# intel/hexl

Hardware: NVIDIA H100
Metric: ntt_per_sec_fwd_inv_N65536_q55_batch8192 (higher is better)
Workload: dtype u64

## Files before the change

### hexl_b200/csrc/ntt.cu

```cuda
#include "ntt_kernels.cuh"

namespace hexl_b200 {
namespace {

template <int MODE, int LOGC>
cudaError_t launch_row(bool fwd, const NttDeviceTables& t, u64* result, const u64* operand,
                       u64 batch, int out_mf, int fold, cudaStream_t stream) {
  using Cfg = RowCfg<LOGC, MODE>;
  const unsigned rows_per_poly = (unsigned)(t.n >> LOGC);
  const u64 total_rows = batch * rows_per_poly;
  const unsigned grid = (unsigned)((total_rows + Cfg::ROWS - 1) / Cfg::ROWS);
  const Mod m = make_mod(t);
  if (fwd) {
    if (cudaError_t e = ensure_dynamic_smem<ntt_row_fwd<MODE, LOGC>>(Cfg::SMEM)) return e;
    ntt_row_fwd<MODE, LOGC><<<grid, Cfg::THREADS, Cfg::SMEM, stream>>>(result, operand, Tab<MODE>::fwd(t), m,
                                                                       total_rows, rows_per_poly, out_mf);
  } else {
    if (cudaError_t e = ensure_dynamic_smem<ntt_row_inv<MODE, LOGC>>(Cfg::SMEM)) return e;
    ntt_row_inv<MODE, LOGC><<<grid, Cfg::THREADS, Cfg::SMEM, stream>>>(
        result, operand, Tab<MODE>::inv(t), m, total_rows, rows_per_poly, out_mf, fold, Tab<MODE>::inv_n(t),
        Tab<MODE>::inv_n_w(t));
  }
  count_launch();
  return cudaGetLastError();
// ... 22 lines not shown
  const unsigned grid = (unsigned)((total_cols + threads - 1) / threads);
  const Mod m = make_mod(t);
  if (fwd)
    ntt_col<MODE, LOGR, true><<<grid, threads, 0, stream>>>(result, operand, Tab<MODE>::fwd(t), m, t.log_n, log_s,
                                                            total_cols, out_mf, fold, Tab<MODE>::inv_n(t),
                                                            Tab<MODE>::inv_n_w(t));
  else
    ntt_col<MODE, LOGR, false><<<grid, threads, 0, stream>>>(result, operand, Tab<MODE>::inv(t), m, t.log_n, log_s,
                                                             total_cols, out_mf, fold, Tab<MODE>::inv_n(t),
                                                             Tab<MODE>::inv_n_w(t));
  count_launch();
  return cudaGetLastError();
}

template <int MODE>
cudaError_t launch_col_dyn(int log_r, bool fwd, const NttDeviceTables& t, u64* result,
                           const u64* operand, u64 batch, int log_s, int out_mf, int fold,
                           cudaStream_t stream) {
  switch (log_r) {
    case 3: return launch_col<MODE, 3>(fwd, t, result, operand, batch, log_s, out_mf, fold, stream);
    case 4: return launch_col<MODE, 4>(fwd, t, result, operand, batch, log_s, out_mf, fold, stream);
  }
  if constexpr (MODE != kSmall)
    if (log_r == 5) return launch_col<MODE, 5>(fwd, t, result, operand, batch, log_s, out_mf, fold, stream);
  return cudaErrorInvalidValue;
}

cudaError_t simple_transform(bool fwd, const NttDeviceTables& t, u64* result, const u64* operand,
                             int out_mf, u64 batch, cudaStream_t stream) {
  const u64 total = batch << (t.log_n - 1);
  const unsigned threads = 128, grid = (unsigned)((total + threads - 1) / threads);
  const u64* src = operand;
  const Mod m = make_mod(t);
  for (int k = 0; k < t.log_n; ++k) {
    const int s = fwd ? k : t.log_n - 1 - k;
    const int last = k == t.log_n - 1;
    if (fwd)
      ntt_stage_simple<true><<<grid, threads, 0, stream>>>(result, src, t.fwd, m, t.log_n, s, total,
                                                           out_mf, last, t.inv_n, t.inv_n_w);
    else
      ntt_stage_simple<false><<<grid, threads, 0, stream>>>(result, src, t.inv, m, t.log_n, s, total,
                                                            out_mf, last, t.inv_n, t.inv_n_w);
    count_launch();
    src = result;
  }
  return cudaGetLastError();
}

template <int MODE, int LOGR>
cudaError_t launch_fused(bool fwd, const NttDeviceTables& t, u64* result, const u64* operand, u64 batch,
                         int out_mf, cudaStream_t stream) {
  using Cfg = FusedCfg<LOGR>;
  const Mod m = make_mod(t);
  cudaLaunchConfig_t cfg = {};
  cfg.gridDim = dim3((unsigned)(batch * Cfg::K));
  cfg.blockDim = dim3(Cfg::THREADS);
  cfg.dynamicSmemBytes = Cfg::SMEM;
  cfg.stream = stream;
  cudaLaunchAttribute attr;
  attr.id = cudaLaunchAttributeClusterDimension;
  attr.val.clusterDim.x = Cfg::K;
  attr.val.clusterDim.y = 1;
  attr.val.clusterDim.z = 1;
  cfg.attrs = &attr;
  cfg.numAttrs = 1;
  cudaError_t e;
  if (fwd)
    e = cudaLaunchKernelEx(&cfg, ntt_fused_fwd<MODE, LOGR>, result, operand, Tab<MODE>::fwd(t), m, out_mf);
  else
    e = cudaLaunchKernelEx(&cfg, ntt_fused_inv<MODE, LOGR>, result, operand, Tab<MODE>::inv(t), m, out_mf,
                           Tab<MODE>::inv_n(t), Tab<MODE>::inv_n_w(t));
  count_launch();
  return e != cudaSuccess ? e : cudaGetLastError();
}

template <int MODE, int LOGR>
cudaError_t launch_pipe(const NttDeviceTables& t, u64* result, const u64* operand, u64 batch, int out_mf,
                        cudaStream_t stream) {
  return launch_pipelined<ntt_pipe_fwd<MODE, LOGR>, PipeCfg<LOGR>>(batch, stream, result, operand, Tab<MODE>::fwd(t),
                                                                  make_mod(t), out_mf);
}

template <int MODE, int LOGR>
cudaError_t launch_dsmem(bool fwd, const NttDeviceTables& t, u64* result, const u64* operand, u64 batch, int out_mf,
                         cudaStream_t stream) {
  using Cfg = DsmemCfg<LOGR, MODE>;
  const Mod m = make_mod(t);
  cudaLaunchConfig_t cfg = {};
  cfg.gridDim = dim3((unsigned)(batch * Cfg::K));
  cfg.blockDim = dim3(Cfg::THREADS);
  cfg.dynamicSmemBytes = Cfg::SMEM;
  cfg.stream = stream;
  cudaLaunchAttribute attr;
  attr.id = cudaLaunchAttributeClusterDimension;
  attr.val.clusterDim.x = Cfg::K;
  attr.val.clusterDim.y = 1;
  attr.val.clusterDim.z = 1;
  cfg.attrs = &attr;
  cfg.numAttrs = 1;
  cudaError_t e;
  if (fwd) {
    if ((e = ensure_dynamic_smem<ntt_dsmem_fwd<MODE, LOGR>>(Cfg::SMEM)) != cudaSuccess) return e;
    e = cudaLaunchKernelEx(&cfg, ntt_dsmem_fwd<MODE, LOGR>, result, operand, Tab<MODE>::fwd(t), m, out_mf);
  } else {
    if ((e = ensure_dynamic_smem<ntt_dsmem_inv<MODE, LOGR>>(Cfg::SMEM)) != cudaSuccess) return e;
    e = cudaLaunchKernelEx(&cfg, ntt_dsmem_inv<MODE, LOGR>, result, operand, Tab<MODE>::inv(t), m, out_mf,
                           Tab<MODE>::inv_n(t), Tab<MODE>::inv_n_w(t));
  }
  count_launch();
  return e != cudaSuccess ? e : cudaGetLastError();
}

enum : int { kSplit, kPipe, kFused, kDsmem };
struct SinglePass {
  int kernel, log_r;
};
template <int MODE>
SinglePass plan_single_pass(int log_n, u64 batch, bool forward) {
  const int lr = log_n - 12;
  if (lr < 2 || lr > 5) return {kSplit, 0};
  if (MODE == kSmall) return {kDsmem, lr};
  if (forward && lr >= 3 && batch >= 64 && batch < (1ull << 31)) return {kPipe, lr};
  if (lr <= 3) return {kDsmem, lr};
  if (lr == 4) return {kFused, lr};
// ... 96 lines not shown
```

### hexl_b200/csrc/ntt_kernels.cuh

```cuda
#pragma once
#include <algorithm>
#include <atomic>
#include <cstdio>
#include <cstdlib>

#include "internal.h"

namespace hexl_b200 {
namespace {

template <int I>
struct Idx {
  __host__ __device__ constexpr operator int() const { return I; }
};
template <int BEGIN, int END, typename F>
__device__ __forceinline__ void static_for(F&& f) {
  if constexpr (BEGIN < END) {
    f(Idx<BEGIN>{});
    static_for<BEGIN + 1, END>(f);
  }
}

enum : int { kGeneric = 0, kFast = 1, kSmall = 2, kWide = 3 };

// ... 146 lines not shown
  return join(t0, t1);
}

template <int MODE, typename TW>
__device__ __forceinline__ void fwd_bfly(u64& X, u64& Y, const TW& w, const Mod& m) {
  if (MODE == kFast) {
    const u64 T = mul_tw<kFast>(Y, w, m);
    Y = X + m.four_q - T;
    X = add_alu(X, T, m);
  } else if (MODE == kWide) {
    const u64 tx = csub(X, m.four_q);
    const u64 T = mul_tw<kWide>(Y, w, m);
    X = add_alu(tx, T, m);
    Y = tx + m.four_q - T;
  } else {
    const u64 tx = csub_s(X, m.two_q);
    const u64 T = mul_tw<kGeneric>(Y, w, m);
    X = tx + T;
    Y = tx + m.two_q - T;
  }
}

template <int MODE, typename TW>
__device__ __forceinline__ void inv_bfly(u64& X, u64& Y, const TW& w, const Mod& m, u64 cq) {
  if (MODE == kFast) {
    const u64 d = X + cq - Y;
    X = add_alu(X, Y, m);
    Y = mul_tw<kFast>(d, w, m);
  } else if (MODE == kWide) {
    const u64 s = add_alu(X, Y, m);
    const u64 d = X + m.four_q - Y;
    X = csub_s(s, m.four_q);
    Y = mul_tw<kWide>(d, w, m);
  } else {
    const u64 s = X + Y;
    const u64 d = X + m.two_q - Y;
    X = csub_s(s, m.two_q);
    Y = mul_tw<kGeneric>(d, w, m);
  }
}

template <int MODE>
__device__ __forceinline__ void inv_bfly_last(u64& X, u64& Y, const Twiddle inv_n, const Twiddle inv_n_w,
                                              const Mod& m, u64 cq) {
  const u64 s = add_alu(X, Y, m);
  const u64 d = X + cq - Y;
  if (MODE == kFast || MODE == kWide) {
    X = mul_tw<MODE>(s, inv_n, m);
    Y = mul_tw<MODE>(d, inv_n_w, m);
  } else {
    X = mul_tw_exact(s, inv_n, m);
    Y = mul_tw_exact(d, inv_n_w, m);
  }
}

template <int MODE>
__device__ __forceinline__ u64 fwd_out(u64 v, const Mod& m, int out_mf) {
  if (MODE == kFast) v = barrett_lazy3_bigq(v, m);
  if (MODE == kWide) v = csub_s(v, m.four_q);
  return out_mf == 1 ? csub_s(csub_s(v, m.two_q), m.q) : v;
}
template <int MODE>
__device__ __forceinline__ u64 inv_out(u64 v, const Mod& m, int out_mf) {
  if (MODE == kFast || MODE == kWide) v = csub_s(v, m.two_q);
  return out_mf == 1 ? csub_s(v, m.q) : v;
}

__device__ __forceinline__ unsigned csub32(unsigned x, unsigned c) { return min(x, x - c); }
__device__ __forceinline__ unsigned mul_tw32(unsigned x, const Twiddle32 w, const Mod& m) {
  const unsigned Q = hi32(mul_wide(x, w.wp));
  return mad_lo(Q, m.n0, x * w.w);
}
template <int MODE, typename TW>
__device__ __forceinline__ void fwd_bfly(unsigned& X, unsigned& Y, const TW& w, const Mod& m) {
  const unsigned two_q = lo32(m.two_q);
  const unsigned tx = csub32(X, two_q);
  const unsigned T = mul_tw32(Y, w, m);
  X = tx + T;
  Y = tx + two_q - T;
}
template <int MODE, typename TW>
__device__ __forceinline__ void inv_bfly(unsigned& X, unsigned& Y, const TW& w, const Mod& m, unsigned) {
  const unsigned two_q = lo32(m.two_q);
  const unsigned s = X + Y;
  const unsigned d = X + two_q - Y;
  X = csub32(s, two_q);
  Y = mul_tw32(d, w, m);
}
template <int MODE>
__device__ __forceinline__ void inv_bfly_last(unsigned& X, unsigned& Y, const Twiddle32 inv_n,
                                              const Twiddle32 inv_n_w, const Mod& m, unsigned) {
  const unsigned s = X + Y;
  const unsigned d = X + lo32(m.two_q) - Y;
  X = mul_tw32(s, inv_n, m);
  Y = mul_tw32(d, inv_n_w, m);
}
template <int MODE>
__device__ __forceinline__ unsigned fwd_out(unsigned v, const Mod& m, int out_mf) {
  return out_mf == 1 ? csub32(csub32(v, lo32(m.two_q)), lo32(m.q)) : v;
}
template <int MODE>
__device__ __forceinline__ unsigned inv_out(unsigned v, const Mod& m, int out_mf) {
  return out_mf == 1 ? csub32(v, lo32(m.q)) : v;
}

__host__ __device__ constexpr int inv_slot_bound(int K, int low) {
// ... 311 lines not shown
        static_for<0, 16>([&](auto I) {
          constexpr int e = I;
          mir->p[p][mir->off + reg_index<LB0>(u, e)] = (u64)inv_out<MODE>(v[e], m, out_mf);
        });
      }
    }
  }
}

template <int MODE, int LOGC>
__global__ void __launch_bounds__(RowCfg<LOGC, MODE>::THREADS, RowCfg<LOGC, MODE>::MIN_BLOCKS)
    ntt_row_fwd(u64* result, const u64* operand, const typename Ar<MODE>::Tw* __restrict__ tw, const Mod m,
                u64 total_rows, unsigned rows_per_poly, int out_mf) {
  using Cfg = RowCfg<LOGC, MODE>;
  extern __shared__ __align__(16) unsigned char smem[];
  const unsigned row_local = threadIdx.x / Cfg::T, u = threadIdx.x % Cfg::T;
  u64 row = (u64)blockIdx.x * Cfg::ROWS + row_local;
  const bool active = row < total_rows;
  if (!active) row = total_rows - 1;
  const u64 base = (u64)rows_per_poly + (row % rows_per_poly);
  typename Cfg::Tw* cta_stab = nullptr;
  if (MODE == kSmall && Cfg::ROWS > 1 && Cfg::TW_TABLES && rows_per_poly == 1)
    cta_stab = reinterpret_cast<typename Cfg::Tw*>(smem + (size_t)row_elems<typename Cfg::E>(LOGC) * sizeof(typename Cfg::E));
  row_fwd_body<MODE, LOGC, kStream, kStream>(
      result + row * Cfg::C, operand + row * Cfg::C,
      reinterpret_cast<typename Cfg::E*>(smem + (size_t)row_local * Cfg::ROW_BYTES), u, base, tw, m, out_mf, active,
      cta_stab);
}

template <int MODE, int LOGC>
__global__ void __launch_bounds__(RowCfg<LOGC, MODE>::THREADS, RowCfg<LOGC, MODE>::MIN_BLOCKS)
    ntt_row_inv(u64* result, const u64* operand, const typename Ar<MODE>::Tw* __restrict__ tw, const Mod m,
                u64 total_rows, unsigned rows_per_poly, int out_mf, int fold, typename Ar<MODE>::Tw inv_n,
                typename Ar<MODE>::Tw inv_n_w) {
  using Cfg = RowCfg<LOGC, MODE>;
  extern __shared__ __align__(16) unsigned char smem[];
  const unsigned row_local = threadIdx.x / Cfg::T, u = threadIdx.x % Cfg::T;
  u64 row = (u64)blockIdx.x * Cfg::ROWS + row_local;
  const bool active = row < total_rows;
  if (!active) row = total_rows - 1;
  const u64 base = (u64)rows_per_poly + (row % rows_per_poly);
  typename Cfg::Tw* cta_stab = nullptr;
  if (MODE == kSmall && Cfg::ROWS > 1 && Cfg::TW_TABLES && rows_per_poly == 1)
    cta_stab = reinterpret_cast<typename Cfg::Tw*>(smem + (size_t)row_elems<typename Cfg::E>(LOGC) * sizeof(typename Cfg::E));
  row_inv_body<MODE, LOGC, kStream, kStream>(
      result + row * Cfg::C, operand + row * Cfg::C,
      reinterpret_cast<typename Cfg::E*>(smem + (size_t)row_local * Cfg::ROW_BYTES), u, base, tw, m, out_mf,
      fold != 0, inv_n, inv_n_w, active, cta_stab);
}

template <int MODE, int LOGR, bool FWD>
__device__ __forceinline__ void col_stages(typename Ar<MODE>::E (&v)[1 << LOGR], const typename Ar<MODE>::Tw* stw,
                                           const Mod& m, bool root_fold, typename Ar<MODE>::Tw inv_n,
                                           typename Ar<MODE>::Tw inv_n_w) {
  using E = typename Ar<MODE>::E;
  using Tw = typename Ar<MODE>::Tw;
  constexpr int R = 1 << LOGR;
  static_for<0, LOGR>([&](auto STEP) {
    constexpr int step = STEP;
    constexpr int s = FWD ? step : LOGR - 1 - step;
    constexpr int eb = LOGR - 1 - s;
    const E cq = stage_cq<MODE>(step, m);
    auto groups = [&] {
      static_for<0, (1 << s)>([&](auto GI) {
        constexpr int gi = GI;
        const Tw w = stw[(1 << s) + gi];
        static_for<0, (1 << eb)>([&](auto L) {
          constexpr int e = (gi << (eb + 1)) | L;
          if constexpr (FWD)
            fwd_bfly<MODE>(v[e], v[e | (1 << eb)], w, m);
          else
            inv_bfly<MODE>(v[e], v[e | (1 << eb)], w, m, cq);
        });
      });
    };
    if constexpr (!FWD && s == 0) {
      if (root_fold) {
        static_for<0, (1 << eb)>([&](auto L) {
          constexpr int l = L;
          inv_bfly_last<MODE>(v[l], v[l | (1 << eb)], inv_n, inv_n_w, m, cq);
        });
      } else {
        groups();
      }
    } else {
      groups();
    }
  });
  if constexpr (!FWD && MODE == kFast) {
    if (!root_fold) inv_pass_fixup<LOGR, R>(v, m);
  }
}

template <int MODE, int LOGR, bool FWD, int LD, int ST>
__device__ __forceinline__ void col_body(u64* result, const u64* operand, u64 off, int log_stride,
                                         const typename Ar<MODE>::Tw* stw, const Mod& m, int out_mf, bool root_fold,
                                         typename Ar<MODE>::Tw inv_n, typename Ar<MODE>::Tw inv_n_w,
                                         const MirrorList* mir = nullptr, bool reduce_in = false) {
  using E = typename Ar<MODE>::E;
  constexpr int R = 1 << LOGR;
  E v[R];
  static_for<0, R>([&](auto I) {
    constexpr int e = I;
    v[e] = (E)ld_coef<LD>(operand + off + ((u64)e << log_stride));
  });
  if constexpr (FWD && sizeof(E) == 8) {
    if (reduce_in) {
      static_for<0, R>([&](auto I) { constexpr int e = I; v[e] = reduce_any(v[e], m); });
    }
  }
  col_stages<MODE, LOGR, FWD>(v, stw, m, root_fold, inv_n, inv_n_w);
  const bool final_out = !FWD && root_fold;
  static_for<0, R>([&](auto I) {
    constexpr int e = I;
    st_coef<ST>(result + off + ((u64)e << log_stride), final_out ? inv_out<MODE>(v[e], m, out_mf) : v[e]);
  });
  if (mir && final_out) {
    for (unsigned p = 0; p < mir->count; ++p) {
      static_for<0, R>([&](auto I) {
        constexpr int e = I;
        mir->p[p][mir->off + off + ((u64)e << log_stride)] = (u64)inv_out<MODE>(v[e], m, out_mf);
      });
    }
  }
}

template <int MODE, int LOGR, bool FWD>
__global__ void __launch_bounds__(256)
    ntt_col(u64* result, const u64* operand, const typename Ar<MODE>::Tw* __restrict__ tw, const Mod m, int log_n,
            int log_s, u64 total_cols, int out_mf, int fold, typename Ar<MODE>::Tw inv_n,
            typename Ar<MODE>::Tw inv_n_w) {
  constexpr int R = 1 << LOGR;
  __shared__ typename Ar<MODE>::Tw stw[R];
  const int log_cols = log_s - LOGR;
  const u64 g0 = (u64)blockIdx.x * blockDim.x;
  const u64 blk = g0 >> log_cols;
  const u64 blocks_per_poly = 1ull << (log_n - log_s);
  const u64 base = blocks_per_poly + (blk & (blocks_per_poly - 1));
  for (int l = threadIdx.x; l < R; l += blockDim.x) {
    if (l == 0) continue;
    const int s = 31 - __clz(l);
    stw[l] = ld_tw(tw + (base << s) + (l - (1 << s)));
  }
  __syncthreads();
  const u64 g = g0 + threadIdx.x;
  if (g >= total_cols) return;
  const u64 c = g & ((1ull << log_cols) - 1);
  col_body<MODE, LOGR, FWD, kStream, kStream>(result, operand, (blk << log_s) + c, log_cols, stw, m, out_mf,
                                              !FWD && fold && log_s == log_n, inv_n, inv_n_w);
}

__device__ __forceinline__ void cluster_barrier() {
  asm volatile("barrier.cluster.arrive.release.aligned;\n\tbarrier.cluster.wait.acquire.aligned;" ::: "memory");
}

template <int LOGR>
struct FusedCfg {
  static constexpr int LOGC = 12, C = 1 << LOGC, R = 1 << LOGR;
  static constexpr int K = R < 8 ? R : 8;
  static constexpr int THREADS = 256;
  static constexpr int MIN_BLOCKS = LOGR <= 4 ? kRowMinBlocks : 2;
  static constexpr size_t SMEM = RowCfg<LOGC>::ROW_BYTES;
};

template <int MODE, int LOGR>
__global__ void __launch_bounds__(FusedCfg<LOGR>::THREADS, FusedCfg<LOGR>::MIN_BLOCKS)
    ntt_fused_fwd(u64* result, const u64* operand, const typename Ar<MODE>::Tw* __restrict__ tw, const Mod m,
                  int out_mf) {
  using Cfg = FusedCfg<LOGR>;
  using E = typename Ar<MODE>::E;
  using Tw = typename Ar<MODE>::Tw;
  extern __shared__ __align__(16) unsigned char smem_raw[];
  E* smem = reinterpret_cast<E*>(smem_raw);
  __shared__ Tw stw[Cfg::R];
  const unsigned rank = blockIdx.x % Cfg::K;
  const u64 poly_off = (u64)(blockIdx.x / Cfg::K) << (Cfg::LOGC + LOGR);
  for (int l = threadIdx.x; l < Cfg::R; l += Cfg::THREADS)
    if (l) stw[l] = ld_tw(tw + l);
  __syncthreads();
  constexpr int COLS = Cfg::C / Cfg::K;
#pragma unroll 1
  for (int c = threadIdx.x; c < COLS; c += Cfg::THREADS)
    col_body<MODE, LOGR, true, kStream, kViaL2>(result, operand, poly_off + rank * COLS + c, Cfg::LOGC, stw, m,
                                                out_mf, false, Tw{}, Tw{});
  cluster_barrier();
#pragma unroll 1
  for (unsigned r = rank; r < Cfg::R; r += Cfg::K) {
    u64* row = result + poly_off + (u64)r * Cfg::C;
    row_fwd_body<MODE, Cfg::LOGC, kViaL2, kStream>(row, row, smem, threadIdx.x, (u64)Cfg::R + r, tw, m, out_mf, true);
    if (r + Cfg::K < Cfg::R) __syncthreads();
  }
}

template <int MODE, int LOGR>
__global__ void __launch_bounds__(FusedCfg<LOGR>::THREADS, FusedCfg<LOGR>::MIN_BLOCKS)
    ntt_fused_inv(u64* result, const u64* operand, const typename Ar<MODE>::Tw* __restrict__ tw, const Mod m,
                  int out_mf, typename Ar<MODE>::Tw inv_n, typename Ar<MODE>::Tw inv_n_w) {
  using Cfg = FusedCfg<LOGR>;
  using E = typename Ar<MODE>::E;
  using Tw = typename Ar<MODE>::Tw;
  extern __shared__ __align__(16) unsigned char smem_raw[];
  E* smem = reinterpret_cast<E*>(smem_raw);
  __shared__ Tw stw[Cfg::R];
  const unsigned rank = blockIdx.x % Cfg::K;
  const u64 poly_off = (u64)(blockIdx.x / Cfg::K) << (Cfg::LOGC + LOGR);
  for (int l = threadIdx.x; l < Cfg::R; l += Cfg::THREADS)
    if (l) stw[l] = ld_tw(tw + l);
#pragma unroll 1
  for (unsigned r = rank; r < Cfg::R; r += Cfg::K) {
    const u64 off = poly_off + (u64)r * Cfg::C;
    row_inv_body<MODE, Cfg::LOGC, kStream, kViaL2>(result + off, operand + off, smem, threadIdx.x, (u64)Cfg::R + r,
                                                   tw, m, out_mf, false, inv_n, inv_n_w, true);
    __syncthreads();
  }
  cluster_barrier();
  constexpr int COLS = Cfg::C / Cfg::K;
#pragma unroll 1
  for (int c = threadIdx.x; c < COLS; c += Cfg::THREADS)
    col_body<MODE, LOGR, false, kViaL2, kStream>(result, result, poly_off + rank * COLS + c, Cfg::LOGC, stw, m,
                                                 out_mf, true, inv_n, inv_n_w);
}

__device__ __forceinline__ unsigned ld_acquire_gpu(const unsigned* p) {
  unsigned v;
  asm volatile("ld.acquire.gpu.global.u32 %0, [%1];" : "=r"(v) : "l"(p) : "memory");
  return v;
}
__device__ __forceinline__ void red_release_gpu(unsigned* p, unsigned v) {
  asm volatile("red.release.gpu.global.add.u32 [%0], %1;" ::"l"(p), "r"(v) : "memory");
}

template <int LOGR>
struct PipeCfg {
  static constexpr int LOGC = 12, C = 1 << LOGC, R = 1 << LOGR;
  static constexpr int THREADS = 256;
  static constexpr int CT = C / THREADS;
  static constexpr int SLOTS = CT + R;
  static constexpr int MIN_BLOCKS = FusedCfg<LOGR>::MIN_BLOCKS;
  static constexpr size_t SMEM = RowCfg<LOGC>::ROW_BYTES;
};

template <int MODE, int LOGR>
__global__ void __launch_bounds__(PipeCfg<LOGR>::THREADS, PipeCfg<LOGR>::MIN_BLOCKS)
    ntt_pipe_fwd(u64* result, const u64* operand, const typename Ar<MODE>::Tw* __restrict__ tw, const Mod m,
                 int out_mf, unsigned batch, unsigned lookahead, unsigned* counter, unsigned* done) {
  using Cfg = PipeCfg<LOGR>;
  using E = typename Ar<MODE>::E;
  using Tw = typename Ar<MODE>::Tw;
  extern __shared__ __align__(16) unsigned char smem_raw[];
  E* smem = reinterpret_cast<E*>(smem_raw);
  __shared__ Tw stw[Cfg::R];
  __shared__ unsigned s_item;
  for (int l = threadIdx.x; l < Cfg::R; l += Cfg::THREADS)
    if (l) stw[l] = ld_tw(tw + l);
  const unsigned total = (batch + lookahead) * Cfg::SLOTS;
  while (true) {
    __syncthreads();
    if (threadIdx.x == 0) s_item = atomicAdd(counter, 1u);
    __syncthreads();
    const unsigned item = s_item;
    if (item >= total) break;
    const unsigned blk = item / Cfg::SLOTS, j = item % Cfg::SLOTS;
    if (j < (unsigned)Cfg::CT) {
      if (blk >= batch) continue;
      const u64 poly_off = (u64)blk << (Cfg::LOGC + LOGR);
      col_body<MODE, LOGR, true, kStream, kViaL2>(result, operand, poly_off + j * Cfg::THREADS + threadIdx.x, Cfg::LOGC,
                                                  stw, m, out_mf, false, Tw{}, Tw{});
      __syncthreads();
      if (threadIdx.x == 0) red_release_gpu(done + blk, 1u);
    } else {
      if (blk < lookahead) continue;
      const unsigned p = blk - lookahead, r = j - Cfg::CT;
      if (threadIdx.x == 0)
        while (ld_acquire_gpu(done + p) < (unsigned)Cfg::CT) __nanosleep(100);
      __syncthreads();
      u64* row = result + ((u64)p << (Cfg::LOGC + LOGR)) + (u64)r * Cfg::C;
      row_fwd_body<MODE, Cfg::LOGC, kViaL2, kStream>(row, row, smem, threadIdx.x, (u64)Cfg::R + r, tw, m, out_mf, true);
    }
  }
}

__device__ __forceinline__ unsigned dsmem_address(const void* local_smem, unsigned cta_rank) {
  const unsigned a = (unsigned)__cvta_generic_to_shared(local_smem);
  unsigned r;
  asm("mapa.shared::cluster.u32 %0, %1, %2;" : "=r"(r) : "r"(a), "r"(cta_rank));
  return r;
}
__device__ __forceinline__ void dsmem_store(unsigned addr, unsigned v) {
  asm volatile("st.shared::cluster.u32 [%0], %1;" ::"r"(addr), "r"(v) : "memory");
}
__device__ __forceinline__ void dsmem_store(unsigned addr, u64 v) {
  asm volatile("st.shared::cluster.u64 [%0], %1;" ::"r"(addr), "l"(v) : "memory");
}
template <typename E>
__device__ __forceinline__ E dsmem_load(unsigned addr) {
  E v;
  if constexpr (sizeof(E) == 8)
    asm volatile("ld.shared::cluster.u64 %0, [%1];" : "=l"(v) : "r"(addr) : "memory");
  else
    asm volatile("ld.shared::cluster.u32 %0, [%1];" : "=r"(v) : "r"(addr) : "memory");
  return v;
}

template <int LOGR, int MODE = kSmall>
struct DsmemCfg {
  using E = typename Ar<MODE>::E;
  using Tw = typename Ar<MODE>::Tw;
  static constexpr int LOGC = 12, C = 1 << LOGC, R = 1 << LOGR;
  static constexpr int K = R < 8 ? R : 8;
  static constexpr int RPC = R / K;
  static constexpr int THREADS = 256;
  static constexpr int COLS = C / K;
  static constexpr bool PAD = sizeof(E) == 8;
  static constexpr int ROW_POLICY = PAD ? kSmemRowPad : kSmemRow;
  static constexpr unsigned ROW = row_elems<E>(LOGC);
  static constexpr size_t SMEM = (size_t)(RPC + (PAD ? 0 : 1)) * ROW * sizeof(E) + kRowTwEntries * sizeof(Tw);
  static constexpr int MIN_BLOCKS = PAD ? kRowMinBlocks : (SMEM <= 56 * 1024 ? 4 : (SMEM <= 75 * 1024 ? 3 : 2));
  static __device__ __forceinline__ unsigned slot(unsigned j) { return PAD ? j + (j >> 4) : j; }
};

template <int MODE, int LOGR>
__global__ void __launch_bounds__(DsmemCfg<LOGR, MODE>::THREADS, DsmemCfg<LOGR, MODE>::MIN_BLOCKS)
    ntt_dsmem_fwd(u64* result, const u64* operand, const typename Ar<MODE>::Tw* __restrict__ tw, const Mod m,
                  int out_mf) {
  using Cfg = DsmemCfg<LOGR, MODE>;
  using E = typename Ar<MODE>::E;
  using Tw = typename Ar<MODE>::Tw;
  extern __shared__ __align__(16) unsigned char smem_raw[];
  E* rows = reinterpret_cast<E*>(smem_raw);
  E* xbuf = rows + Cfg::RPC * Cfg::ROW;
  Tw* const ctab = Cfg::PAD ? reinterpret_cast<Tw*>(xbuf) : nullptr;
  __shared__ Tw stw[Cfg::R];
  const unsigned rank = blockIdx.x % Cfg::K;
  const u64 poly_off = (u64)(blockIdx.x / Cfg::K) << (Cfg::LOGC + LOGR);
  asm volatile("barrier.cluster.arrive.relaxed.aligned;" ::: "memory");
  for (int l = threadIdx.x; l < Cfg::R; l += Cfg::THREADS)
    if (l) stw[l] = ld_tw(tw + l);
  __syncthreads();
  asm volatile("barrier.cluster.wait.aligned;" ::: "memory");
  unsigned owner_base[Cfg::K];
  static_for<0, Cfg::K>([&](auto I) { constexpr int o = I; owner_base[o] = dsmem_address(rows, o); });
#pragma unroll 1
  for (int c = threadIdx.x; c < Cfg::COLS; c += Cfg::THREADS) {
    const unsigned col = rank * Cfg::COLS + c;
    E v[Cfg::R];
    static_for<0, Cfg::R>([&](auto I) {
      constexpr int e = I;
      v[e] = (E)ld_coef<kStream>(operand + poly_off + ((u64)e << Cfg::LOGC) + col);
    });
    col_stages<MODE, LOGR, true>(v, stw, m, false, Tw{}, Tw{});
    static_for<0, Cfg::R>([&](auto I) {
      constexpr int e = I;
      dsmem_store(owner_base[e % Cfg::K] + ((e / Cfg::K) * Cfg::ROW + Cfg::slot(col)) * (unsigned)sizeof(E), v[e]);
    });
  }
  cluster_barrier();
#pragma unroll 1
  for (int lr = 0; lr < Cfg::RPC; ++lr) {
    const unsigned r = rank + lr * Cfg::K;
    E* row = rows + lr * Cfg::ROW;
    row_fwd_body<MODE, Cfg::LOGC, Cfg::ROW_POLICY, kStream>(result + poly_off + (u64)r * Cfg::C, row,
                                                            Cfg::PAD ? row : xbuf, threadIdx.x, (u64)Cfg::R + r, tw, m,
                                                            out_mf, true, ctab);
    if (lr + 1 < Cfg::RPC) __syncthreads();
  }
}

template <int MODE, int LOGR>
__global__ void __launch_bounds__(DsmemCfg<LOGR, MODE>::THREADS, DsmemCfg<LOGR, MODE>::MIN_BLOCKS)
    ntt_dsmem_inv(u64* result, const u64* operand, const typename Ar<MODE>::Tw* __restrict__ tw, const Mod m,
                  int out_mf, typename Ar<MODE>::Tw inv_n, typename Ar<MODE>::Tw inv_n_w) {
  using Cfg = DsmemCfg<LOGR, MODE>;
  using E = typename Ar<MODE>::E;
  using Tw = typename Ar<MODE>::Tw;
  extern __shared__ __align__(16) unsigned char smem_raw[];
  E* rows = reinterpret_cast<E*>(smem_raw);
  E* xbuf = rows + Cfg::RPC * Cfg::ROW;
  Tw* const ctab = Cfg::PAD ? reinterpret_cast<Tw*>(xbuf) : nullptr;
  __shared__ Tw stw[Cfg::R];
  const unsigned rank = blockIdx.x % Cfg::K;
  const u64 poly_off = (u64)(blockIdx.x / Cfg::K) << (Cfg::LOGC + LOGR);
  for (int l = threadIdx.x; l < Cfg::R; l += Cfg::THREADS)
    if (l) stw[l] = ld_tw(tw + l);
#pragma unroll 1
  for (int lr = 0; lr < Cfg::RPC; ++lr) {
    const unsigned r = rank + lr * Cfg::K;
    E* row = rows + lr * Cfg::ROW;
    row_inv_body<MODE, Cfg::LOGC, kStream, Cfg::ROW_POLICY>(row, operand + poly_off + (u64)r * Cfg::C,
                                                            Cfg::PAD ? row : xbuf, threadIdx.x, (u64)Cfg::R + r, tw, m,
                                                            out_mf, false, inv_n, inv_n_w, true, ctab);
    __syncthreads();
  }
  cluster_barrier();
  unsigned owner_base[Cfg::K];
  static_for<0, Cfg::K>([&](auto I) { constexpr int o = I; owner_base[o] = dsmem_address(rows, o); });
#pragma unroll 1
  for (int c = threadIdx.x; c < Cfg::COLS; c += Cfg::THREADS) {
    const unsigned col = rank * Cfg::COLS + c;
    E v[Cfg::R];
    static_for<0, Cfg::R>([&](auto I) {
      constexpr int e = I;
      v[e] = dsmem_load<E>(owner_base[e % Cfg::K] + ((e / Cfg::K) * Cfg::ROW + Cfg::slot(col)) * (unsigned)sizeof(E));
    });
    col_stages<MODE, LOGR, false>(v, stw, m, true, inv_n, inv_n_w);
    static_for<0, Cfg::R>([&](auto I) {
      constexpr int e = I;
      st_coef<kStream>(result + poly_off + ((u64)e << Cfg::LOGC) + col, inv_out<MODE>(v[e], m, out_mf));
    });
  }
  cluster_barrier();
}

template <bool FWD>
__global__ void ntt_stage_simple(u64* result, const u64* src, const Twiddle* __restrict__ tw,
                                 const Mod m, int log_n, int s ,
                                 u64 total_bflies, int out_mf, int last, Twiddle inv_n,
                                 Twiddle inv_n_w) {
  const u64 g = (u64)blockIdx.x * blockDim.x + threadIdx.x;
  if (g >= total_bflies) return;
  const int log_t = log_n - 1 - s;
  const u64 half = 1ull << (log_n - 1);
  const u64 poly = g >> (log_n - 1), k = g & (half - 1);
  const u64 i = k >> log_t, jj = k & ((1ull << log_t) - 1);
  const u64 j = (poly << log_n) + (i << (log_t + 1)) + jj;
  u64 X = src[j], Y = src[j + (1ull << log_t)];
  if (FWD) {
    fwd_bfly<kGeneric>(X, Y, ld_tw(tw + (1ull << s) + i), m);
    if (last) {
      X = fwd_out<kGeneric>(X, m, out_mf);
      Y = fwd_out<kGeneric>(Y, m, out_mf);
    }
  } else if (last) {
    inv_bfly_last<kGeneric>(X, Y, inv_n, inv_n_w, m, m.two_q);
    X = inv_out<kGeneric>(X, m, out_mf);
    Y = inv_out<kGeneric>(Y, m, out_mf);
  } else {
    inv_bfly<kGeneric>(X, Y, ld_tw(tw + (1ull << s) + i), m, m.two_q);
  }
  result[j] = X;
  result[j + (1ull << log_t)] = Y;
}


template <auto Kernel>
cudaError_t ensure_dynamic_smem(size_t bytes) {
  if (bytes <= 48 * 1024) return cudaSuccess;
  static std::atomic<unsigned long long> done{0};
  int dev = 0;
  cudaGetDevice(&dev);
  const unsigned long long bit = 1ull << (dev & 63);
  if (done.load(std::memory_order_acquire) & bit) return cudaSuccess;
  const cudaError_t e = cudaFuncSetAttribute(Kernel, cudaFuncAttributeMaxDynamicSharedMemorySize, (int)bytes);
  if (e == cudaSuccess) done.fetch_or(bit, std::memory_order_release);
  return e;
}

template <auto Kernel, typename Cfg, typename... Args>
cudaError_t launch_pipelined(u64 units, cudaStream_t stream, Args... args) {
  static const unsigned lookahead = [] {
    const char* v = std::getenv("HEXL_B200_PIPE_LOOKAHEAD");
    return (unsigned)std::max(1, v ? std::atoi(v) : 16);
  }();
  cudaError_t e = ensure_dynamic_smem<Kernel>(Cfg::SMEM);
  if (e != cudaSuccess) return e;
  int dev = 0, sms = 0;
  cudaGetDevice(&dev);
  cudaDeviceGetAttribute(&sms, cudaDevAttrMultiProcessorCount, dev);
  const u64 items = (units + lookahead) * Cfg::SLOTS;
  const unsigned grid = (unsigned)std::min<u64>((u64)sms * Cfg::MIN_BLOCKS, items);
  unsigned* state = nullptr;
  const size_t bytes = (size_t)(units + 1) * sizeof(unsigned);
  if ((e = scratch_alloc_async(reinterpret_cast<void**>(&state), bytes, stream)) != cudaSuccess) return e;
  if ((e = cudaMemsetAsync(state, 0, bytes, stream)) == cudaSuccess) {
    Kernel<<<grid, Cfg::THREADS, Cfg::SMEM, stream>>>(args..., (unsigned)units, lookahead, state, state + 1);
    count_launch();
    e = cudaGetLastError();
  }
  scratch_free_async(state, stream);
  return e;
}

inline int pick_mode(u64 q) {
  if (q < kSmallModulusLimit) return kSmall;
  if (q < kFastModulusLimit && q >= (1ull << 32)) return kFast;
  return (q >= kFastModulusLimit && q < kWideModulusLimit) ? kWide : kGeneric;
}

template <int MODE>
struct Tab {
  static const Twiddle* fwd(const NttDeviceTables& t) { return t.fwd; }
  static const Twiddle* inv(const NttDeviceTables& t) { return t.inv; }
  static Twiddle inv_n(const NttDeviceTables& t) { return t.inv_n; }
  static Twiddle inv_n_w(const NttDeviceTables& t) { return t.inv_n_w; }
};
template <>
struct Tab<kSmall> {
  static const Twiddle32* fwd(const NttDeviceTables& t) { return t.fwd32; }
  static const Twiddle32* inv(const NttDeviceTables& t) { return t.inv32; }
  static Twiddle32 inv_n(const NttDeviceTables& t) { return t.inv_n32; }
  static Twiddle32 inv_n_w(const NttDeviceTables& t) { return t.inv_n_w32; }
};

__host__ __device__ inline Mod make_mod(u64 q, u64 mu) {
  Mod m;
  m.q = q;
  m.two_q = q << 1;
  m.four_q = q << 2;
  m.mu = mu;
  const u64 negq = 0 - q;
  m.n0 = (unsigned)negq;
  m.n1 = (unsigned)(negq >> 32);
  m.zero = 0;
  return m;
}
// ... 17 lines not shown
```

### hexl_b200/csrc/ntt_multi.cu

```cuda
#include "ntt_kernels.cuh"

namespace hexl_b200 {
namespace {

__device__ __forceinline__ NttDeviceParams load_params(const NttMulti& multi, u64 poly) {
  return *multi.p[poly / multi.group];
}

template <int MODE, int LOGC, bool FWD, bool MUL = false>
__global__ void __launch_bounds__(RowCfg<LOGC, MODE>::THREADS, RowCfg<LOGC, MODE>::MIN_BLOCKS)
    ntt_row_multi(u64* result, const u64* operand, const __grid_constant__ NttMulti multi, u64 total_rows,
                  unsigned rows_per_poly, int out_mf, int fold, unsigned gather) {
  using Cfg = RowCfg<LOGC, MODE>;
  extern __shared__ __align__(16) unsigned char smem[];
  const unsigned row_local = threadIdx.x / Cfg::T, u = threadIdx.x % Cfg::T;
  u64 row = (u64)blockIdx.x * Cfg::ROWS + row_local;
  const bool active = row < total_rows;
  if (!active) row = total_rows - 1;
  const NttDeviceParams P = load_params(multi, row / rows_per_poly);
  const Mod m = make_mod(P.q, P.mu);
  const u64 base = (u64)rows_per_poly + (row % rows_per_poly);
  typename Cfg::E* srow = reinterpret_cast<typename Cfg::E*>(smem + (size_t)row_local * Cfg::ROW_BYTES);
  if (FWD) {
    const u64 poly = row / rows_per_poly;
    const u64 src_row = gather ? (poly % gather) * rows_per_poly + row % rows_per_poly : row;
    row_fwd_body<MODE, LOGC, kStream, kStream>(result + row * Cfg::C, operand + src_row * Cfg::C, srow, u, base, P.fwd, m,
                                               out_mf, active, nullptr, gather != 0);
  } else {
    const MirrorList mir{multi.mirror, multi.mirrors, row * Cfg::C};
    const ProdIn prod{MUL ? multi.mul + row * Cfg::C : nullptr, P.prod_mu, P.prod_shift};
    row_inv_body<MODE, LOGC, kStream, kStream>(result + row * Cfg::C, operand + row * Cfg::C, srow, u, base, P.inv, m,
                                               out_mf, fold != 0, P.inv_n, P.inv_n_w, active, nullptr,
                                               &mir, MUL ? &prod : nullptr);
  }
}

template <int MODE, int LOGR, bool FWD>
__global__ void __launch_bounds__(256)
    ntt_col_multi(u64* result, const u64* operand, const __grid_constant__ NttMulti multi, int log_n, int log_s,
                  u64 total_cols, int out_mf, int fold, unsigned gather) {
  constexpr int R = 1 << LOGR;
  __shared__ Twiddle stw[R];
  const int log_cols = log_s - LOGR;
  const u64 g0 = (u64)blockIdx.x * blockDim.x;
  const u64 blk = g0 >> log_cols;
  const u64 blocks_per_poly = 1ull << (log_n - log_s);
  const NttDeviceParams P = load_params(multi, blk >> (log_n - log_s));
  const Mod m = make_mod(P.q, P.mu);
  const Twiddle* tw = FWD ? P.fwd : P.inv;
  const u64 base = blocks_per_poly + (blk & (blocks_per_poly - 1));
  for (int l = threadIdx.x; l < R; l += blockDim.x) {
    if (l == 0) continue;
    const int s = 31 - __clz(l);
    stw[l] = ld_tw(tw + (base << s) + (l - (1 << s)));
  }
  __syncthreads();
  const u64 g = g0 + threadIdx.x;
  if (g >= total_cols) return;
  const u64 c = g & ((1ull << log_cols) - 1);
  const MirrorList mir{multi.mirror, multi.mirrors, 0};
  const u64 poly = blk >> (log_n - log_s);
  const u64* src = (FWD && gather) ? operand + (((poly % gather) - poly) << log_n) : operand;
  col_body<MODE, LOGR, FWD, kStream, kStream>(result, src, (blk << log_s) + c, log_cols, stw, m, out_mf,
                                              !FWD && fold && log_s == log_n, P.inv_n, P.inv_n_w,
                                              FWD ? nullptr : &mir, FWD && gather != 0);
}

template <int MODE, int LOGR>
__global__ void __launch_bounds__(PipeCfg<LOGR>::THREADS, PipeCfg<LOGR>::MIN_BLOCKS)
    ntt_pipe_multi(u64* result, const u64* operand, const __grid_constant__ NttMulti multi, int out_mf, unsigned units,
                   unsigned lookahead, unsigned* counter, unsigned* done) {
  using Cfg = PipeCfg<LOGR>;
  using E = typename Ar<MODE>::E;
  extern __shared__ __align__(16) unsigned char smem_raw[];
  E* smem = reinterpret_cast<E*>(smem_raw);
  __shared__ Twiddle stw[Cfg::R];
  __shared__ unsigned s_item;
  const unsigned total = (units + lookahead) * Cfg::SLOTS;
  unsigned staged = ~0u;
  while (true) {
    __syncthreads();
    if (threadIdx.x == 0) s_item = atomicAdd(counter, 1u);
    __syncthreads();
    const unsigned item = s_item;
    if (item >= total) break;
    const unsigned blk = item / Cfg::SLOTS, j = item % Cfg::SLOTS;
    const bool producer = j < (unsigned)Cfg::CT;
    if (producer ? blk >= units : blk < lookahead) continue;
    const unsigned poly = producer ? blk : blk - lookahead;
    const unsigned entry = poly / multi.group;
    const NttDeviceParams P = *multi.p[entry];
    const Mod m = make_mod(P.q, P.mu);
    if (entry != staged) {
      for (int l = threadIdx.x; l < Cfg::R; l += Cfg::THREADS)
        if (l) stw[l] = ld_tw(P.fwd + l);
      staged = entry;
      __syncthreads();
    }
    const u64 poly_off = (u64)poly << (Cfg::LOGC + LOGR);
    if (!producer) {
      if (threadIdx.x == 0)
        while (ld_acquire_gpu(done + poly) < (unsigned)Cfg::CT) __nanosleep(100);
      __syncthreads();
    }
    if (producer) {
      col_body<MODE, LOGR, true, kStream, kViaL2>(result, operand, poly_off + j * Cfg::THREADS + threadIdx.x, Cfg::LOGC,
                                                  stw, m, out_mf, false, Twiddle{}, Twiddle{});
    } else {
      const unsigned r = j - Cfg::CT;
      u64* row = result + poly_off + (u64)r * Cfg::C;
      row_fwd_body<MODE, Cfg::LOGC, kViaL2, kStream>(row, row, smem, threadIdx.x, (u64)Cfg::R + r, P.fwd, m, out_mf,
                                                     true);
    }
    if (producer) {
      __syncthreads();
      if (threadIdx.x == 0) red_release_gpu(done + poly, 1u);
    }
  }
}

template <bool FWD, int LOGN>
__global__ void ntt_tiny_multi(u64* result, const u64* operand, const __grid_constant__ NttMulti multi, u64 units,
                               int out_mf) {
  const u64 unit = (u64)blockIdx.x * blockDim.x + threadIdx.x;
  if (unit >= units) return;
  const NttDeviceParams P = *multi.p[unit / multi.group];
  const Mod m = make_mod(P.q, P.mu);
  constexpr int n = 1 << LOGN;
  u64 v[n];
  const u64 src_unit = (FWD && multi.gather) ? unit % multi.gather : unit;
  static_for<0, n>([&](auto I) {
    constexpr int e = I;
    v[e] = operand[src_unit * n + e];
    if (FWD && multi.gather) v[e] %= P.q;
    if (!FWD && multi.mul) v[e] = prod_lazy<kGeneric>(v[e], multi.mul[unit * n + e], m, P.prod_mu, P.prod_shift);
  });
  static_for<0, LOGN>([&](auto K) {
    constexpr int k = K;
    constexpr int s = FWD ? k : LOGN - 1 - k;
    constexpr int t = n >> (s + 1);
    static_for<0, (1 << s)>([&](auto I) {
      constexpr int i = I;
      static_for<0, t>([&](auto J) {
        constexpr int j = J;
        u64& X = v[2 * i * t + j];
        u64& Y = v[2 * i * t + j + t];
        if constexpr (FWD)
          fwd_bfly<kGeneric>(X, Y, P.fwd[(1 << s) + i], m);
        else if constexpr (s == 0)
          inv_bfly_last<kGeneric>(X, Y, P.inv_n, P.inv_n_w, m, m.two_q);
        else
          inv_bfly<kGeneric>(X, Y, P.inv[(1 << s) + i], m, m.two_q);
      });
    });
  });
  static_for<0, n>([&](auto I) {
    constexpr int e = I;
    result[unit * n + e] = FWD ? fwd_out<kGeneric>(v[e], m, out_mf) : inv_out<kGeneric>(v[e], m, out_mf);
  });
  if (!FWD)
// ... 138 lines not shown
```

Measured before the change: 1.481 million.

## Pipeline inverse fused NTT via persistent work queue and cheaper root-fold scaling

The cluster-based fused inverse NTT kernel becomes a persistent, atomic-counter-driven pipelined kernel. Row passes for one polynomial act as producers, and column passes for a polynomial a lookahead of 32 earlier consume them once a release/acquire done-counter fills. This mirrors the existing forward pipeline and removes the cluster barrier. It also adds a specialized root butterfly that multiplies the sum branch by n^{-1} with a shift-based Montgomery-like trick instead of a full twiddle multiply. The risks are spin-wait stalls, L2 residency depending on lookahead, and correctness of the new inverse-n reduction.

```diff
diff --git a/hexl_b200/csrc/ntt.cu b/hexl_b200/csrc/ntt.cu
--- a/hexl_b200/csrc/ntt.cu
+++ b/hexl_b200/csrc/ntt.cu
@@ -98,6 +98,9 @@
                          int out_mf, cudaStream_t stream) {
   using Cfg = FusedCfg<LOGR>;
   const Mod m = make_mod(t);
+  if (!fwd)
+    return launch_pipelined<ntt_fused_inv<MODE, LOGR>, PipeCfg<LOGR, false>>(
+        batch, stream, result, operand, Tab<MODE>::inv(t), m, out_mf, Tab<MODE>::inv_n(t), Tab<MODE>::inv_n_w(t));
   cudaLaunchConfig_t cfg = {};
   cfg.gridDim = dim3((unsigned)(batch * Cfg::K));
   cfg.blockDim = dim3(Cfg::THREADS);
@@ -110,12 +113,8 @@
   attr.val.clusterDim.z = 1;
   cfg.attrs = &attr;
   cfg.numAttrs = 1;
-  cudaError_t e;
-  if (fwd)
-    e = cudaLaunchKernelEx(&cfg, ntt_fused_fwd<MODE, LOGR>, result, operand, Tab<MODE>::fwd(t), m, out_mf);
-  else
-    e = cudaLaunchKernelEx(&cfg, ntt_fused_inv<MODE, LOGR>, result, operand, Tab<MODE>::inv(t), m, out_mf,
-                           Tab<MODE>::inv_n(t), Tab<MODE>::inv_n_w(t));
+  const cudaError_t e = cudaLaunchKernelEx(&cfg, ntt_fused_fwd<MODE, LOGR>, result, operand, Tab<MODE>::fwd(t), m,
+                                           out_mf);
   count_launch();
   return e != cudaSuccess ? e : cudaGetLastError();
 }
diff --git a/hexl_b200/csrc/ntt_kernels.cuh b/hexl_b200/csrc/ntt_kernels.cuh
--- a/hexl_b200/csrc/ntt_kernels.cuh
+++ b/hexl_b200/csrc/ntt_kernels.cuh
@@ -222,6 +222,18 @@
     X = mul_tw_exact(s, inv_n, m);
     Y = mul_tw_exact(d, inv_n_w, m);
   }
+}
+template <int MODE>
+__device__ __forceinline__ void inv_bfly_root(u64& X, u64& Y, const Twiddle inv_n, const Twiddle inv_n_w, int log_n,
+                                              const Mod& m, u64 cq) {
+  const u64 s = add_alu(X, Y, m);
+  const u64 d = X + cq - Y;
+  const unsigned k = (0u - lo32(s)) & ((1u << log_n) - 1u);
+  unsigned c0, c1, t0, t1;
+  split(m.q - inv_n.w, c0, c1);
+  split(mad_wide(k, c0, add_alu(s, (u64)k, m) >> log_n), t0, t1);
+  X = join(t0, mad_lo(k, c1, t1));
+  Y = (MODE == kFast || MODE == kWide) ? mul_tw<MODE>(d, inv_n_w, m) : mul_tw_exact(d, inv_n_w, m);
 }
 
 template <int MODE>
@@ -639,7 +651,7 @@
 template <int MODE, int LOGR, bool FWD>
 __device__ __forceinline__ void col_stages(typename Ar<MODE>::E (&v)[1 << LOGR], const typename Ar<MODE>::Tw* stw,
                                            const Mod& m, bool root_fold, typename Ar<MODE>::Tw inv_n,
-                                           typename Ar<MODE>::Tw inv_n_w) {
+                                           typename Ar<MODE>::Tw inv_n_w, int log_n) {
   using E = typename Ar<MODE>::E;
   using Tw = typename Ar<MODE>::Tw;
   constexpr int R = 1 << LOGR;
@@ -665,7 +677,10 @@
       if (root_fold) {
         static_for<0, (1 << eb)>([&](auto L) {
           constexpr int l = L;
-          inv_bfly_last<MODE>(v[l], v[l | (1 << eb)], inv_n, inv_n_w, m, cq);
+          if constexpr (sizeof(E) == 8)
+            inv_bfly_root<MODE>(v[l], v[l | (1 << eb)], inv_n, inv_n_w, log_n, m, cq);
+          else
+            inv_bfly_last<MODE>(v[l], v[l | (1 << eb)], inv_n, inv_n_w, m, cq);
         });
       } else {
         groups();
@@ -682,7 +697,7 @@
 template <int MODE, int LOGR, bool FWD, int LD, int ST>
 __device__ __forceinline__ void col_body(u64* result, const u64* operand, u64 off, int log_stride,
                                          const typename Ar<MODE>::Tw* stw, const Mod& m, int out_mf, bool root_fold,
-                                         typename Ar<MODE>::Tw inv_n, typename Ar<MODE>::Tw inv_n_w,
+                                         typename Ar<MODE>::Tw inv_n, typename Ar<MODE>::Tw inv_n_w, int log_n,
                                          const MirrorList* mir = nullptr, bool reduce_in = false) {
   using E = typename Ar<MODE>::E;
   constexpr int R = 1 << LOGR;
@@ -696,7 +711,7 @@
       static_for<0, R>([&](auto I) { constexpr int e = I; v[e] = reduce_any(v[e], m); });
     }
   }
-  col_stages<MODE, LOGR, FWD>(v, stw, m, root_fold, inv_n, inv_n_w);
+  col_stages<MODE, LOGR, FWD>(v, stw, m, root_fold, inv_n, inv_n_w, log_n);
   const bool final_out = !FWD && root_fold;
   static_for<0, R>([&](auto I) {
     constexpr int e = I;
@@ -734,7 +749,7 @@
   if (g >= total_cols) return;
   const u64 c = g & ((1ull << log_cols) - 1);
   col_body<MODE, LOGR, FWD, kStream, kStream>(result, operand, (blk << log_s) + c, log_cols, stw, m, out_mf,
-                                              !FWD && fold && log_s == log_n, inv_n, inv_n_w);
+                                              !FWD && fold && log_s == log_n, inv_n, inv_n_w, log_n);
 }
 
 __device__ __forceinline__ void cluster_barrier() {
@@ -769,7 +784,7 @@
 #pragma unroll 1
   for (int c = threadIdx.x; c < COLS; c += Cfg::THREADS)
     col_body<MODE, LOGR, true, kStream, kViaL2>(result, operand, poly_off + rank * COLS + c, Cfg::LOGC, stw, m,
-                                                out_mf, false, Tw{}, Tw{});
+                                                out_mf, false, Tw{}, Tw{}, Cfg::LOGC + LOGR);
   cluster_barrier();
 #pragma unroll 1
   for (unsigned r = rank; r < Cfg::R; r += Cfg::K) {
@@ -779,35 +794,6 @@
   }
 }
 
-template <int MODE, int LOGR>
-__global__ void __launch_bounds__(FusedCfg<LOGR>::THREADS, FusedCfg<LOGR>::MIN_BLOCKS)
-    ntt_fused_inv(u64* result, const u64* operand, const typename Ar<MODE>::Tw* __restrict__ tw, const Mod m,
-                  int out_mf, typename Ar<MODE>::Tw inv_n, typename Ar<MODE>::Tw inv_n_w) {
-  using Cfg = FusedCfg<LOGR>;
-  using E = typename Ar<MODE>::E;
-  using Tw = typename Ar<MODE>::Tw;
-  extern __shared__ __align__(16) unsigned char smem_raw[];
-  E* smem = reinterpret_cast<E*>(smem_raw);
-  __shared__ Tw stw[Cfg::R];
-  const unsigned rank = blockIdx.x % Cfg::K;
-  const u64 poly_off = (u64)(blockIdx.x / Cfg::K) << (Cfg::LOGC + LOGR);
-  for (int l = threadIdx.x; l < Cfg::R; l += Cfg::THREADS)
-    if (l) stw[l] = ld_tw(tw + l);
-#pragma unroll 1
-  for (unsigned r = rank; r < Cfg::R; r += Cfg::K) {
-    const u64 off = poly_off + (u64)r * Cfg::C;
-    row_inv_body<MODE, Cfg::LOGC, kStream, kViaL2>(result + off, operand + off, smem, threadIdx.x, (u64)Cfg::R + r,
-                                                   tw, m, out_mf, false, inv_n, inv_n_w, true);
-    __syncthreads();
-  }
-  cluster_barrier();
-  constexpr int COLS = Cfg::C / Cfg::K;
-#pragma unroll 1
-  for (int c = threadIdx.x; c < COLS; c += Cfg::THREADS)
-    col_body<MODE, LOGR, false, kViaL2, kStream>(result, result, poly_off + rank * COLS + c, Cfg::LOGC, stw, m,
-                                                 out_mf, true, inv_n, inv_n_w);
-}
-
 __device__ __forceinline__ unsigned ld_acquire_gpu(const unsigned* p) {
   unsigned v;
   asm volatile("ld.acquire.gpu.global.u32 %0, [%1];" : "=r"(v) : "l"(p) : "memory");
@@ -817,7 +803,9 @@
   asm volatile("red.release.gpu.global.add.u32 [%0], %1;" ::"l"(p), "r"(v) : "memory");
 }
 
-template <int LOGR>
+constexpr int kPipeInvLookahead = 32;
+
+template <int LOGR, bool FWD = true>
 struct PipeCfg {
   static constexpr int LOGC = 12, C = 1 << LOGC, R = 1 << LOGR;
   static constexpr int THREADS = 256;
@@ -825,6 +813,7 @@
   static constexpr int SLOTS = CT + R;
   static constexpr int MIN_BLOCKS = FusedCfg<LOGR>::MIN_BLOCKS;
   static constexpr size_t SMEM = RowCfg<LOGC>::ROW_BYTES;
+  static constexpr int LOOKAHEAD = FWD ? 16 : kPipeInvLookahead;
 };
 
 template <int MODE, int LOGR>
@@ -852,7 +841,7 @@
       if (blk >= batch) continue;
       const u64 poly_off = (u64)blk << (Cfg::LOGC + LOGR);
       col_body<MODE, LOGR, true, kStream, kViaL2>(result, operand, poly_off + j * Cfg::THREADS + threadIdx.x, Cfg::LOGC,
-                                                  stw, m, out_mf, false, Tw{}, Tw{});
+                                                  stw, m, out_mf, false, Tw{}, Tw{}, Cfg::LOGC + LOGR);
       __syncthreads();
       if (threadIdx.x == 0) red_release_gpu(done + blk, 1u);
     } else {
@@ -863,6 +852,48 @@
       __syncthreads();
       u64* row = result + ((u64)p << (Cfg::LOGC + LOGR)) + (u64)r * Cfg::C;
       row_fwd_body<MODE, Cfg::LOGC, kViaL2, kStream>(row, row, smem, threadIdx.x, (u64)Cfg::R + r, tw, m, out_mf, true);
+    }
+  }
+}
+
+template <int MODE, int LOGR>
+__global__ void __launch_bounds__(PipeCfg<LOGR, false>::THREADS, PipeCfg<LOGR, false>::MIN_BLOCKS)
+    ntt_fused_inv(u64* result, const u64* operand, const typename Ar<MODE>::Tw* __restrict__ tw, const Mod m,
+                  int out_mf, typename Ar<MODE>::Tw inv_n, typename Ar<MODE>::Tw inv_n_w, unsigned batch,
+                  unsigned lookahead, unsigned* counter, unsigned* done) {
+  using Cfg = PipeCfg<LOGR, false>;
+  using E = typename Ar<MODE>::E;
+  using Tw = typename Ar<MODE>::Tw;
+  extern __shared__ __align__(16) unsigned char smem_raw[];
+  E* smem = reinterpret_cast<E*>(smem_raw);
+  __shared__ Tw stw[Cfg::R];
+  __shared__ unsigned s_item;
+  for (int l = threadIdx.x; l < Cfg::R; l += Cfg::THREADS)
+    if (l) stw[l] = ld_tw(tw + l);
+  const unsigned total = (batch + lookahead) * Cfg::SLOTS;
+  while (true) {
+    __syncthreads();
+    if (threadIdx.x == 0) s_item = atomicAdd(counter, 1u);
+    __syncthreads();
+    const unsigned item = s_item;
+    if (item >= total) break;
+    const unsigned blk = item / Cfg::SLOTS, j = item % Cfg::SLOTS;
+    if (j < (unsigned)Cfg::R) {
+      if (blk >= batch) continue;
+      const u64 off = ((u64)blk << (Cfg::LOGC + LOGR)) + (u64)j * Cfg::C;
+      row_inv_body<MODE, Cfg::LOGC, kStream, kViaL2>(result + off, operand + off, smem, threadIdx.x, (u64)Cfg::R + j,
+                                                     tw, m, out_mf, false, inv_n, inv_n_w, true);
+      __syncthreads();
+      if (threadIdx.x == 0) red_release_gpu(done + blk, 1u);
+    } else {
+      if (blk < lookahead) continue;
+      const unsigned p = blk - lookahead;
+      if (threadIdx.x == 0)
+        while (ld_acquire_gpu(done + p) < (unsigned)Cfg::R) __nanosleep(100);
+      __syncthreads();
+      const u64 poly_off = (u64)p << (Cfg::LOGC + LOGR);
+      col_body<MODE, LOGR, false, kViaL2, kStream>(result, result, poly_off + (j - Cfg::R) * Cfg::THREADS + threadIdx.x,
+                                                   Cfg::LOGC, stw, m, out_mf, true, inv_n, inv_n_w, Cfg::LOGC + LOGR);
     }
   }
 }
@@ -935,7 +966,7 @@
       constexpr int e = I;
       v[e] = (E)ld_coef<kStream>(operand + poly_off + ((u64)e << Cfg::LOGC) + col);
     });
-    col_stages<MODE, LOGR, true>(v, stw, m, false, Tw{}, Tw{});
+    col_stages<MODE, LOGR, true>(v, stw, m, false, Tw{}, Tw{}, Cfg::LOGC + LOGR);
     static_for<0, Cfg::R>([&](auto I) {
       constexpr int e = I;
       dsmem_store(owner_base[e % Cfg::K] + ((e / Cfg::K) * Cfg::ROW + Cfg::slot(col)) * (unsigned)sizeof(E), v[e]);
@@ -989,7 +1020,7 @@
       constexpr int e = I;
       v[e] = dsmem_load<E>(owner_base[e % Cfg::K] + ((e / Cfg::K) * Cfg::ROW + Cfg::slot(col)) * (unsigned)sizeof(E));
     });
-    col_stages<MODE, LOGR, false>(v, stw, m, true, inv_n, inv_n_w);
+    col_stages<MODE, LOGR, false>(v, stw, m, true, inv_n, inv_n_w, Cfg::LOGC + LOGR);
     static_for<0, Cfg::R>([&](auto I) {
       constexpr int e = I;
       st_coef<kStream>(result + poly_off + ((u64)e << Cfg::LOGC) + col, inv_out<MODE>(v[e], m, out_mf));
@@ -1046,7 +1077,7 @@
 cudaError_t launch_pipelined(u64 units, cudaStream_t stream, Args... args) {
   static const unsigned lookahead = [] {
     const char* v = std::getenv("HEXL_B200_PIPE_LOOKAHEAD");
-    return (unsigned)std::max(1, v ? std::atoi(v) : 16);
+    return (unsigned)std::max(1, v ? std::atoi(v) : Cfg::LOOKAHEAD);
   }();
   cudaError_t e = ensure_dynamic_smem<Kernel>(Cfg::SMEM);
   if (e != cudaSuccess) return e;
diff --git a/hexl_b200/csrc/ntt_multi.cu b/hexl_b200/csrc/ntt_multi.cu
--- a/hexl_b200/csrc/ntt_multi.cu
+++ b/hexl_b200/csrc/ntt_multi.cu
@@ -62,7 +62,7 @@
   const u64 poly = blk >> (log_n - log_s);
   const u64* src = (FWD && gather) ? operand + (((poly % gather) - poly) << log_n) : operand;
   col_body<MODE, LOGR, FWD, kStream, kStream>(result, src, (blk << log_s) + c, log_cols, stw, m, out_mf,
-                                              !FWD && fold && log_s == log_n, P.inv_n, P.inv_n_w,
+                                              !FWD && fold && log_s == log_n, P.inv_n, P.inv_n_w, log_n,
                                               FWD ? nullptr : &mir, FWD && gather != 0);
 }
 
@@ -105,7 +105,7 @@
     }
     if (producer) {
       col_body<MODE, LOGR, true, kStream, kViaL2>(result, operand, poly_off + j * Cfg::THREADS + threadIdx.x, Cfg::LOGC,
-                                                  stw, m, out_mf, false, Twiddle{}, Twiddle{});
+                                                  stw, m, out_mf, false, Twiddle{}, Twiddle{}, Cfg::LOGC + LOGR);
     } else {
       const unsigned r = j - Cfg::CT;
       u64* row = result + poly_off + (u64)r * Cfg::C;
```

New measurement: 1.506 million (median of 6 runs). 1.7% higher.
